# zhuzhui-2000/mobilesuperresolution

Measured on AMD Instinct MI355X. Metric: HR megapixels/sec (WDSR-B x4, 48x48 LR patches), full training step, higher is better.
Workload: dtype bf16; 1 GPU; WDSR-B x4, 16 blocks / 24 units, 48x48 LR patches, batch 32 per GPU, fwd+L1+bwd+Adam; global_batch=32, parallelism=dp1

## Files before the change

include/sr_hotpath.h:

```cpp
#ifndef SR_HOTPATH_H
#define SR_HOTPATH_H
#include <stddef.h>
#include <stdint.h>

#ifdef __cplusplus
extern "C" {
#endif

typedef void* sr_stream_t;

#define SR_DTYPE_F32 0
#define SR_DTYPE_BF16 1

int sr_abi_version(void);

int sr_wdsr_block_fwd(const void* x, void* y, const void* wblob, const float* cinit,
                      int N, int H, int W, int F, int dtype, sr_stream_t stream);

int sr_wdsr_block2_fwd(const void* x, void* ya, void* yb, const void* wblob_a, const void* wblob_b,
                       const float* cinit_a, const float* cinit_b, void* tsave_a, void* tsave_b, int N, int H, int W,
                       int F, int dtype, sr_stream_t stream);

int sr_wdsr_block2_bwd_data(const void* xa, const void* xb, const void* dyb, void* dxb, void* dxa,
                            const void* wblob_a, const void* wblob_b, const float* cinit_a, const float* cinit_b,
// ... 152 lines not shown
  const float* flat; float* gflat;
  const int* chan_tab; int n_chan;
  const int* bias_tab; const float* bias_const; int n_bias;
  float* src; float* dsrc;
  long src_head_off, src_body_off, src_body_stride, src_tail_off;
  const int* idx_head; int n_idx_head;
  const int* idx_body; int n_idx_body;
  const int* idx_cinit; int n_idx_cinit;
  const int* idx_tail; int n_idx_tail;
  void* blob_head; void* blob_body; float* cinit_body; void* blob_tail;
  float* part_a; float* part_b; float* part_tail; float* part_head;
  int wgs_body, wgs_tail, wgs_head;
  int slab_a, slab_b, slab_tail, slab_head;
  const int* ga_sidx; const int* ga_dst; int n_ga;
  const int* gb_sidx; const int* gb_dst; int n_gb;
  const int* gt_sidx; const int* gt_dst; int n_gt;
  const int* gh_sidx; const int* gh_dst; int n_gh;
  const float* x; void* acts; void* grads; float* out; const float* dout;
  void* tsave; void* dtsave;
  const float* hr; int loss_kind; float loss_gscale; float* loss_part;
  int nb_split, chan_split, bias_split;
  int adam_in_wn_bwd;
  int one_block32;
} sr_wdsr_net_t;

#define SR_NET_SAVE_ACTS 1
#define SR_NET_WEIGHTS_PACKED 2
#define SR_NET_PACK_ONLY 4
int sr_wdsr_net_forward(const sr_wdsr_net_t* net, int flags, sr_stream_t stream);
int sr_wdsr_net_backward(const sr_wdsr_net_t* net, sr_stream_t stream);
int sr_wdsr_net_backward_part(const sr_wdsr_net_t* net, int part, sr_stream_t stream);

int sr_pixel_shuffle(const float* in, float* out, int N, int C, int H, int W, int r, int inverse, sr_stream_t stream);

int sr_tail_bwd_loss(const float* sr, const float* hr, int loss_kind, float gscale, float* loss_part, const void* feat,
                     const float* x_nchw, float mean, const void* wblob, void* dfeat, float* partial, int wgs, int N, int H,
                     int W, int F, int R, int dtype, sr_stream_t stream);

typedef struct { float w_lerp, beta2, one_minus_beta2, bc2_sqrt, eps, neg_step_size; } sr_adam_t;
int sr_adam_step(float* param, const float* grad, float* exp_avg, float* exp_avg_sq, long n, const sr_adam_t* a,
                 const float* loss_part, int n_loss, float loss_scale, float* loss_out, sr_stream_t stream);
int sr_loss_value(const float* loss_part, int n_loss, float loss_scale, float* loss_out, sr_stream_t stream);
int sr_scale_by(void* y, const void* x, long n, const float* scale, int dtype, sr_stream_t stream);
int sr_wdsr_net_train_step(const sr_wdsr_net_t* net, float* exp_avg, float* exp_avg_sq, long n_params, const sr_adam_t* a,
                           float loss_scale, float* loss_out, sr_stream_t stream);

int sr_conv7_fwd(const void* x, const void* wpacked, const float* bias, void* y, int N, int H, int W, int CIN, int COUT, int relu,
                 int out_f32, sr_stream_t stream);

int sr_probe_mfma_bf16(const void* a_frag, const void* b_frag, float* acc_out, sr_stream_t stream);
int sr_probe_mfma_f32(const float* a_frag, const float* b_frag, float* acc_out, sr_stream_t stream);
int sr_probe_tr_read(const void* img_bf16, int n_elems, const int* lane_elem_off, void* out_bf16x4,
                     sr_stream_t stream);
int sr_probe_copy(const void* src, void* dst, size_t n_bytes, sr_stream_t stream);
int sr_probe_launch_floor(void* out, int gx, int gy, int threads, int lds_bytes, int reps, sr_stream_t stream);
int sr_probe_launch_floor_graph(void* out, int gx, int gy, int threads, int lds_bytes, int reps, int iters,
                                float* us_per_launch, float* host_us_per_graph );
int sr_debug_set_stamps(void* buf, long n_workgroups);

#ifdef __cplusplus
}
#endif
#endif
```

mobilesuperresolution_amd/_lib.py:

```python
from __future__ import annotations

import ctypes
import os
from ctypes import c_int, c_size_t, c_void_p

import torch

_HERE = os.path.dirname(os.path.abspath(__file__))
LIB_PATH = os.environ.get("SR_HOTPATH_LIB_PATH") or os.path.join(
    _HERE, "libsr_hotpath_dbg.so" if os.environ.get("SR_HOTPATH_DEBUG_LIB") == "1" else "libsr_hotpath.so")
ABI_VERSION = 17
DTYPE_CODE = {torch.float32: 0, torch.bfloat16: 1}

_P, _I, _Z, _L, _F = c_void_p, c_int, c_size_t, ctypes.c_long, ctypes.c_float
SIGNATURES = {
    "sr_abi_version": ([], _I),
    "sr_wdsr_block_fwd": ([_P, _P, _P, _P, _I, _I, _I, _I, _I, _P], _I),
    "sr_wdsr_block2_fwd": ([_P] * 9 + [_I] * 5 + [_P], _I),
    "sr_wdsr_fwd_rs": ([_P] * 9 + [_I] * 6 + [_P], _I),
    "sr_conv7_fwd": ([_P] * 4 + [_I] * 7 + [_P], _I),
    "sr_wdsr_fwd_rs_repeat": ([_P] * 9 + [_I] * 7 + [_P], _I),
    "sr_wdsr_block_wgrad_saved": ([_P] * 8 + [_I] * 7 + [_L] * 5 + [_P], _I),
    "sr_wdsr_block2_bwd_data": ([_P] * 11 + [_I] * 5 + [_P], _I),
    "sr_wdsr_block2_fwd_repeat": ([_P] * 7 + [_I] * 6 + [_P], _I),
    "sr_probe_launch_floor": ([_P, _I, _I, _I, _I, _I, _P], _I),
    "sr_probe_launch_floor_graph": ([_P, _I, _I, _I, _I, _I, _I, _P, _P], _I),
    "sr_debug_set_stamps": ([_P, _L], _I),
    "sr_c3_trunk_fwd": ([_P] * 6 + [_I] * 7 + [_L, _P], _I),
    "sr_c3_trunk_bwd": ([_P] * 11 + [_I] * 8 + [_L, _P], _I),
    "sr_c64_trunk_fwd": ([_P] * 7 + [_I] * 7 + [_L, _P], _I),
    "sr_tail_bwd": ([_P, _P, _P, _F, _P, _P, _P] + [_I] * 7 + [_P], _I),
    "sr_nas_dw_wgrad": ([_P, _P, _P, _P, _I, _I, _I, _I, _I, _I, _P], _I),
    "sr_wdsr_block_fwd_repeat": ([_P, _P, _P, _P, _I, _I, _I, _I, _I, _I, _P], _I),
    "sr_wdsr_block_bwd_data": ([_P, _P, _P, _P, _P, _I, _I, _I, _I, _I, _P], _I),
# ... 8 lines not shown
    "sr_c3_bwd_data": ([_P, _P, _P, _P, _P, _I, _I, _I, _I, _I, _I, _P], _I),
    "sr_c3_wgrad": ([_P, _P, _P, _P, _I, _I, _I, _I, _I, _I, _I, _P], _I),
    "sr_flow_warp_fwd": ([_P, _P, _P, _I, _I, _I, _I, _P], _I),
    "sr_flow_warp_bwd": ([_P, _P, _P, _P, _P, _I, _I, _I, _I, _P], _I),
    "sr_nas_dw_fwd": ([_P, _P, _P, _I, _I, _I, _I, _I, _P], _I),
    "sr_nas_pw_fwd": ([_P, _P, _P, _P, _P, _P, _I, _I, _I, _I, _I, _P], _I),
    "sr_nas_pw_bwd": ([_P, _P, _P, _P, _P, _P, _P, _P, _I, _I, _I, _I, _I, _I, _P], _I),
    "sr_nas_dw_bwd": ([_P, _P, _P, _P, _P, _P, _I, _I, _I, _I, _I, _I, _P], _I),
    "sr_patch_gather": ([_P, _P, _P, _P, _I, _I, _I, _P], _I),
    "sr_clip_gather": ([_P] * 7 + [_I] * 4 + [_P], _I),
    "sr_param_pack": ([_P, _P, _P, _I, _P, _P, _I, _P, _I, _I, _P], _I),
    "sr_param_grads": ([_P, _P, _P, _P, _I, _P, _I, _P, _I, _P], _I),
    "sr_nas_scalars": ([_P] * 5 + [_I, _I, _P, _P, _L, _I, _P, _P], _I),
    "sr_nas_mask_grads": ([_P, _L, _I, _I, _I, _I, _P, _P, _P, _I, _I, _P, _P], _I),
    "sr_nas_body_fwd": ([_P, _P, _P, _L, _P, _L, _P, _L, _P, _L] + [_I] * 7 + [_P], _I),
    "sr_nas_body_bwd": ([_P] * 7 + [_L, _P, _L, _P, _L, _P, _L, _P, _L, _P, _L] + [_I] * 8 + [_P, _P], _I),
    "sr_psnr": ([_P, _P, _P, _P] + [_I] * 7 + [_P], _I),
    "sr_pixel_shuffle": ([_P, _P, _I, _I, _I, _I, _I, _I, _P], _I),
    "sr_tail_bwd_loss": ([_P, _P, _I, _F, _P, _P, _P, _F, _P, _P, _P] + [_I] * 7 + [_P], _I),
    "sr_adam_step": ([_P, _P, _P, _P, _L, _P, _P, _I, _F, _P, _P], _I),
    "sr_loss_value": ([_P, _I, _F, _P, _P], _I),
    "sr_scale_by": ([_P, _P, _L, _P, _I, _P], _I),
    "sr_wdsr_net_train_step": ([_P, _P, _P, _L, _P, _F, _P, _P], _I),
    "sr_wdsr_net_forward": ([_P, _I, _P], _I),
    "sr_wdsr_net_backward": ([_P, _P], _I),
    "sr_wdsr_net_backward_part": ([_P, _I, _P], _I),
    "sr_probe_mfma_bf16": ([_P, _P, _P, _P], _I),
    "sr_probe_mfma_f32": ([_P, _P, _P, _P], _I),
    "sr_probe_tr_read": ([_P, _I, _P, _P, _P], _I),
    "sr_probe_copy": ([_P, _P, _Z, _P], _I),
    "sr_rm_block_fwd": ([_P] * 5 + [_I] * 6 + [_P], _I),
    "sr_rm_block_bwd_data": ([_P] * 4 + [_I] * 6 + [_P], _I),
    "sr_rm_wgrad": ([_P] * 4 + [_I] * 8 + [_P], _I),
    "sr_rm_tail_fwd": ([_P] * 3 + [_I] * 7 + [_P], _I),
    "sr_rm_unshuffle": ([_P, _P] + [_I] * 5 + [_P], _I),
    "sr_rm_tail_bwd_data": ([_P] * 3 + [_I] * 7 + [_P], _I),
}

class WdsrNet(ctypes.Structure):
    _fields_ = (
        [(n, _I) for n in ("F", "NB", "R", "dtype", "N", "H", "W")] + [("mean", _F)] +
        [("flat", _P), ("gflat", _P), ("chan_tab", _P), ("n_chan", _I),
         ("bias_tab", _P), ("bias_const", _P), ("n_bias", _I), ("src", _P), ("dsrc", _P)] +
        [(n, _L) for n in ("src_head_off", "src_body_off", "src_body_stride", "src_tail_off")] +
        [("idx_head", _P), ("n_idx_head", _I), ("idx_body", _P), ("n_idx_body", _I),
         ("idx_cinit", _P), ("n_idx_cinit", _I), ("idx_tail", _P), ("n_idx_tail", _I),
         ("blob_head", _P), ("blob_body", _P), ("cinit_body", _P), ("blob_tail", _P),
         ("part_a", _P), ("part_b", _P), ("part_tail", _P), ("part_head", _P)] +
        [(n, _I) for n in ("wgs_body", "wgs_tail", "wgs_head", "slab_a", "slab_b", "slab_tail", "slab_head")] +
        [("ga_sidx", _P), ("ga_dst", _P), ("n_ga", _I), ("gb_sidx", _P), ("gb_dst", _P), ("n_gb", _I),
         ("gt_sidx", _P), ("gt_dst", _P), ("n_gt", _I), ("gh_sidx", _P), ("gh_dst", _P), ("n_gh", _I),
         ("x", _P), ("acts", _P), ("grads", _P), ("out", _P), ("dout", _P), ("tsave", _P), ("dtsave", _P),
         ("hr", _P), ("loss_kind", _I), ("loss_gscale", _F), ("loss_part", _P),
         ("nb_split", _I), ("chan_split", _I), ("bias_split", _I), ("adam_in_wn_bwd", _I),
         ("one_block32", _I)])


class C3Warp(ctypes.Structure):
    _fields_ = [("frame", _P), ("frame_bs", _L), ("state", _P), ("flow", _P), ("flow_bs", _L), ("flow_bound", _P),
                ("dstate", _P), ("dflow", _P), ("dflow_bs", _L), ("x0_save", _P)]


class C3Unpack(ctypes.Structure):
    _fields_ = [("sidx0", _P), ("dst0", _P), ("n0", _I), ("sidx1", _P), ("dst1", _P), ("n1", _I), ("gflat", _P)]


class PackSeg(ctypes.Structure):
    _fields_ = [("idx", _P), ("out", _P), ("src_off", _L), ("src_stride", _L), ("n", _I), ("reps", _I), ("as_float", _I)]


class UnpackSeg(ctypes.Structure):
    _fields_ = [("partial", _P), ("sidx", _P), ("dst", _P), ("dst_off", _L), ("dst_stride", _L), ("slab", _L), ("wgs", _I),
                ("n", _I), ("reps", _I)]


class AdamScalars(ctypes.Structure):
    _fields_ = [(n, _F) for n in ("w_lerp", "beta2", "one_minus_beta2", "bc2_sqrt", "eps", "neg_step_size")]

# ... 102 lines not shown
```

mobilesuperresolution_amd/csrc/sr_abi.hip:

```cpp
#include <algorithm>
#include "../../include/sr_hotpath.h"
#include "wdsr_block.h"
#include "wdsr_fwd_rs.h"
#include "wdsr_fwd_stream.h"
#include "wdsr_bwd_rs.h"
#include "wdsr_bwd_pair_lds.h"
#include "wdsr_wgrad_rs.h"
#include "wdsr_ends.h"
#include "wdsr_prep.h"
#include "conv3x3.h"
#include "conv64.h"
#include "spynet_conv.h"
#include "nas_block.h"
#include "nas_dw_lc.h"
#include "nas_bwd_fused.h"
#include "flow_warp.h"
#include "metrics.h"
#include "patches.h"
#include "clips.h"
#include "train_step.h"
#include "pixel_shuffle.h"
#include "result_block.h"

extern "C" int sr_abi_version(void) { return 17; }

namespace {

template <typename T, int F, int E, int L>
int launch_block_fwd(const void* x, void* y, const void* wblob, const float* cinit, int N, int H, int W,
                     hipStream_t st, void* tsave = nullptr) {
  typedef BlockCfg<F, E, L> C;
  const int tiles_x = (W + C::TW - 1) / C::TW, tiles_y = (H + C::TH - 1) / C::TH;
  dim3 grid(tiles_x * tiles_y, N), block(64 * C::NPT_H);
  hipLaunchKernelGGL((wdsr_block_fwd_kernel<T, F, E, L>), grid, block, 0, st, (const T*)x, (T*)y, (const T*)wblob,
                     cinit, H, W, tiles_x, (T*)tsave);
  SR_HIP_CHECK_LAUNCH();
  return 0;
}

template <typename T, int F, int E, int L>
int launch_block_bwd_data(const void* x, const void* dy, void* dx, const void* wblob, const float* cinit, int N,
                          int H, int W, hipStream_t st, void* dtsave = nullptr) {
  typedef BlockCfg<F, E, L> C;
  const int tiles_x = (W + C::TW - 1) / C::TW, tiles_y = (H + C::TH - 1) / C::TH;
  dim3 grid(tiles_x * tiles_y, N), block(64 * C::NPT_O);
  hipLaunchKernelGGL((wdsr_block_bwd_data_kernel<T, F, E, L>), grid, block, 0, st, (const T*)x, (const T*)dy, (T*)dx,
                     (const T*)wblob, cinit, H, W, tiles_x, (T*)dtsave);
// ... 857 lines not shown
        return rc;
      cur = nxt;
      continue;
    }
    if (save_acts && saved) {
      rc = n->F == 24 ? launch_block_fwd<__bf16, 24, 144, 20>(cur, nxt, (char*)n->blob_body + i * blob,
                                                              n->cinit_body + (size_t)i * n->n_idx_cinit, n->N, n->H, n->W,
                                                              st, (char*)n->tsave + (size_t)i * side)
                      : launch_block_fwd<__bf16, 32, 192, 26>(cur, nxt, (char*)n->blob_body + i * blob,
                                                              n->cinit_body + (size_t)i * n->n_idx_cinit, n->N, n->H, n->W,
                                                              st, (char*)n->tsave + (size_t)i * side);
      if (rc) return rc;
    } else if ((rc = sr_wdsr_block_fwd(cur, nxt, (char*)n->blob_body + i * blob,
                                       n->cinit_body + (size_t)i * n->n_idx_cinit, n->N, n->H, n->W, n->F, n->dtype, stream)))
      return rc;
    cur = nxt;
  }
  return sr_tail_fwd(cur, n->x, n->out, n->blob_tail, n->mean, n->N, n->H, n->W, n->F, n->R, n->dtype, stream);
}

namespace {
struct FusedAdam { float* m; float* v; AdamArgs a; const float* loss_part; int n_loss; float loss_scale; float* loss_out; };
}
static int net_backward_part_impl(const sr_wdsr_net_t* n, int part, sr_stream_t stream, const FusedAdam* fa) {
  if (!n || !n->flat || !n->gflat || !n->dsrc || !n->x || !n->acts || !n->grads || part < 0 || part > 2) return -2;
  if (part != 2 && (n->hr ? (!n->out || !n->loss_part || (n->loss_kind != 1 && n->loss_kind != 2)) : !n->dout)) return -2;
  hipStream_t st = (hipStream_t)stream;
  const size_t esz = n->dtype == SR_DTYPE_BF16 ? 2 : 4;
  const size_t act = (size_t)n->N * n->H * n->W * n->F * esz;
  const size_t blob = (size_t)n->n_idx_body * esz;
  const long act_e = (long)n->N * n->H * n->W * n->F;
  char* acts = (char*)n->acts;
  char* grads = (char*)n->grads;
  const bool pairs = net_uses_pairs(n);
  const bool saved = net_saves_side_images(n, true);
  const size_t side = side_image_bytes(n);
  int split = part == 0 ? 0 : n->nb_split;
  if (part != 0 && (split <= 0 || split >= n->NB || (pairs && ((n->NB - split) & 1)))) return -2;
  const int b0 = part == 1 ? split : 0, b1 = part == 2 ? split : n->NB;
  int rc;
  if (part != 2) {
    if (n->hr) {
      if ((rc = sr_tail_bwd_loss(n->out, n->hr, n->loss_kind, n->loss_gscale, n->loss_part, acts + (size_t)n->NB * act, n->x,
                                 n->mean, n->blob_tail, grads + (size_t)n->NB * act, n->part_tail, n->wgs_tail, n->N, n->H, n->W,
                                 n->F, n->R, n->dtype, stream)))
        return rc;
// ... 41 lines not shown
      return rc;
  }
  const int nl = b1 - b0;
  const int wgs_part = nl > 0 ? (n->wgs_body * n->NB) / nl : 0;
  if (nl > 0) {
    char* a0 = acts + (size_t)b0 * act;
    char* g1 = grads + (size_t)(b0 + 1) * act;
    char* wb0 = (char*)n->blob_body + (size_t)b0 * blob;
    const float* ci0 = n->cinit_body + (size_t)b0 * n->n_idx_cinit;
    float* pa0 = n->part_a;
    float* pb0 = n->part_b;
    if (saved) {
      if ((rc = sr_wdsr_block_wgrad_saved(a0, g1, (char*)n->tsave + (size_t)b0 * side, (char*)n->dtsave + (size_t)b0 * side, wb0, ci0,
                                          pa0, pb0, nl, wgs_part, n->N, n->H, n->W, n->F, n->dtype, act_e, act_e,
                                          (long)(side / esz), (long)n->n_idx_body, (long)n->n_idx_cinit, stream)))
        return rc;
    } else if ((rc = sr_wdsr_block_wgrad(a0, g1, wb0, ci0, pa0, pb0, nl, wgs_part, n->N, n->H, n->W, n->F, n->dtype, act_e,
                                         act_e, (long)n->n_idx_body, (long)n->n_idx_cinit, stream)))
      return rc;
  }
  if (part != 1)
    if ((rc = sr_head_wgrad(grads, n->x, n->mean, n->part_head, n->wgs_head, n->N, n->H, n->W, n->F, n->dtype, stream)))
      return rc;
  {
    UnpackSegs us;
    us.nseg = 0;
    int blk = 0;
    auto add = [&](const float* part_, const int* sidx, const int* dst, long off, long stride, long slab, int wgs, int cnt,
                   int reps) {
      us.s[us.nseg++] = UnpackSeg{part_, sidx, dst, off, stride, slab, wgs, cnt, reps, blk};
      blk += reps * unpack_blocks(cnt, wgs);
    };
    if (nl > 0) {
      add(n->part_a, n->ga_sidx, n->ga_dst, n->src_body_off + b0 * n->src_body_stride, n->src_body_stride, n->slab_a, wgs_part,
          n->n_ga, nl);
      add(n->part_b, n->gb_sidx, n->gb_dst, n->src_body_off + b0 * n->src_body_stride, n->src_body_stride, n->slab_b, wgs_part,
          n->n_gb, nl);
    }
    if (part != 2) add(n->part_tail, n->gt_sidx, n->gt_dst, n->src_tail_off, 0, n->slab_tail, n->wgs_tail, n->n_gt, 1);
    if (part != 1) add(n->part_head, n->gh_sidx, n->gh_dst, n->src_head_off, 0, n->slab_head, n->wgs_head, n->n_gh, 1);
    hipLaunchKernelGGL(unpack_all_kernel, dim3(blk), dim3(64 * UNPACK_Q), 0, st, n->dsrc, us);
  }
  const int c0 = part == 1 ? n->chan_split : 0, c1 = part == 2 ? n->chan_split : n->n_chan;
  const int d0 = part == 1 ? n->bias_split : 0, d1 = part == 2 ? n->bias_split : n->n_bias;
  const int cb = (c1 - c0 + 3) / 4, bb = (d1 - d0 + 255) / 256;
  if (fa)
    hipLaunchKernelGGL(wn_bwd_adam_kernel, dim3(cb + bb), dim3(256), 0, st, const_cast<float*>(n->flat), n->dsrc, n->gflat, fa->m, fa->v,
                       (const int4*)n->chan_tab + c0, c1 - c0, n->bias_tab + 3 * d0, d1 - d0, cb, fa->a, fa->loss_part, fa->n_loss,
                       fa->loss_scale, fa->loss_out);
  else
    hipLaunchKernelGGL(wn_bwd_kernel, dim3(cb + bb), dim3(256), 0, st, n->flat, n->dsrc, n->gflat, (const int4*)n->chan_tab + c0,
                       c1 - c0, n->bias_tab + 3 * d0, d1 - d0, cb);
  SR_HIP_CHECK_LAUNCH();
  return 0;
}
extern "C" int sr_wdsr_net_backward_part(const sr_wdsr_net_t* n, int part, sr_stream_t stream) {
  return net_backward_part_impl(n, part, stream, nullptr);
}

extern "C" int sr_wdsr_net_backward(const sr_wdsr_net_t* n, sr_stream_t stream) { return sr_wdsr_net_backward_part(n, 0, stream); }

extern "C" int sr_param_pack(const float* flat, float* src, const int* chan_tab, int n_chan, const int* bias_tab,
                             const float* bias_const, int n_bias, const sr_pack_seg_t* segs, int nseg, int dtype,
                             sr_stream_t stream) {
  if (!flat || !src || !chan_tab || n_chan <= 0 || n_bias < 0 || (n_bias > 0 && (!bias_tab || !bias_const)) || !segs || nseg < 1 ||
      nseg > 4 || (dtype != SR_DTYPE_F32 && dtype != SR_DTYPE_BF16))
    return -2;
  hipStream_t st = (hipStream_t)stream;
  const int cb = (n_chan + 3) / 4, bb = (n_bias + 255) / 256;
  hipLaunchKernelGGL(wn_src_kernel, dim3(cb + bb), dim3(256), 0, st, flat, src, (const int4*)chan_tab, n_chan, bias_tab, bias_const,
                     n_bias, cb);
  PackSegs ps;
  ps.nseg = nseg;
  int blk = 0;
  for (int k = 0; k < nseg; ++k) {
    const sr_pack_seg_t& g = segs[k];
    if (!g.idx || !g.out || g.n <= 0 || g.reps <= 0) return -2;
// ... 210 lines not shown
extern "C" int sr_scale_by(void* y, const void* x, long n, const float* scale, int dtype, sr_stream_t stream) {
  if (!y || !x || !scale || n <= 0 || ((uintptr_t)y & 15) || ((uintptr_t)x & 15)) return -2;
  const unsigned blocks = (unsigned)((n + 2047) / 2048);
  if (dtype == SR_DTYPE_BF16)
    hipLaunchKernelGGL(scale_by_kernel<__bf16>, dim3(blocks), dim3(256), 0, (hipStream_t)stream, (__bf16*)y, (const __bf16*)x, n, scale);
  else if (dtype == SR_DTYPE_F32)
    hipLaunchKernelGGL(scale_by_kernel<float>, dim3(blocks), dim3(256), 0, (hipStream_t)stream, (float*)y, (const float*)x, n, scale);
  else return -1;
  SR_HIP_CHECK_LAUNCH();
  return 0;
}
extern "C" int sr_wdsr_net_train_step(const sr_wdsr_net_t* n, float* m, float* v, long n_params, const sr_adam_t* a,
                                      float loss_scale, float* loss_out, sr_stream_t stream) {
  if (!n || !n->hr || !m || !v || !a || n_params <= 0) return -2;
  int rc;
  if ((rc = sr_wdsr_net_forward(n, SR_NET_SAVE_ACTS, stream))) return rc;
  if (n->adam_in_wn_bwd) {
    const FusedAdam fa{m, v, AdamArgs{a->w_lerp, a->beta2, a->one_minus_beta2, a->bc2_sqrt, a->eps, a->neg_step_size}, n->loss_part,
                       n->wgs_tail, loss_scale, loss_out};
    return net_backward_part_impl(n, 0, stream, &fa);
  }
  if ((rc = sr_wdsr_net_backward(n, stream))) return rc;
  return sr_adam_step(const_cast<float*>(n->flat), n->gflat, m, v, n_params, a, n->loss_part, n->wgs_tail, loss_scale, loss_out, stream);
}

__global__ void probe_mfma_bf16_kernel(const bf16x8* a, const bf16x8* b, float* out) {
  const int l = threadIdx.x;
  f32x16 acc = zero16();
  acc = mma16<__bf16>(a[l], b[l], acc);
#pragma unroll
  for (int i = 0; i < 16; ++i) out[l * 16 + i] = acc[i];
}
__global__ void probe_mfma_f32_kernel(const f32x8* a, const f32x8* b, float* out) {
  const int l = threadIdx.x;
  f32x16 acc = zero16();
  acc = mma16<float>(a[l], b[l], acc);
#pragma unroll
  for (int i = 0; i < 16; ++i) out[l * 16 + i] = acc[i];
}
__global__ void probe_tr_kernel(const __bf16* img, int n, const int* off, bf16x4* out) {
  __shared__ __attribute__((aligned(16))) __bf16 lds[8192];
  for (int i = threadIdx.x; i < n && i < 8192; i += 64) lds[i] = img[i];
  __syncthreads();
  typedef __attribute__((address_space(3))) bf16x4 lds_bf16x4;
  out[threadIdx.x] = __builtin_amdgcn_ds_read_tr16_b64_v4bf16((lds_bf16x4*)(lds + off[threadIdx.x]));
}
// ... 258 lines not shown
```

mobilesuperresolution_amd/csrc/train_step.h:

```cpp
#pragma once
#include "sr_common.h"

struct AdamArgs {
  float w_lerp, beta2, one_minus_beta2, bc2_sqrt, eps, neg_step_size;
};
__global__ __launch_bounds__(256) void adam_step_kernel(float* __restrict__ p, const float* __restrict__ g,
                                                        float* __restrict__ m, float* __restrict__ v, long n, AdamArgs a,
                                                        const float* __restrict__ loss_part, int n_loss, float loss_scale,
                                                        float* __restrict__ loss_out) {
  const long i0 = ((long)blockIdx.x * 256 + threadIdx.x) * 4;
  if (i0 + 3 < n) {
    const f32x4 gv = *reinterpret_cast<const f32x4*>(g + i0);
    f32x4 mv = *reinterpret_cast<const f32x4*>(m + i0), vv = *reinterpret_cast<const f32x4*>(v + i0);
    f32x4 pv = *reinterpret_cast<const f32x4*>(p + i0);
#pragma unroll
    for (int j = 0; j < 4; ++j) {
      mv[j] = __builtin_fmaf(a.w_lerp, gv[j] - mv[j], mv[j]);
      const float vb = vv[j] * a.beta2;
      vv[j] = __builtin_fmaf(a.one_minus_beta2, gv[j] * gv[j], vb);
      const float d = __builtin_sqrtf(vv[j]) / a.bc2_sqrt + a.eps;
      pv[j] = __builtin_fmaf(a.neg_step_size, mv[j] / d, pv[j]);
    }
    *reinterpret_cast<f32x4*>(m + i0) = mv;
    *reinterpret_cast<f32x4*>(v + i0) = vv;
// ... 30 lines not shown
template <typename T>
__global__ __launch_bounds__(256) void scale_by_kernel(T* __restrict__ y, const T* __restrict__ x, long n, const float* __restrict__ scale) {
  const float s = *scale;
  const long i0 = ((long)blockIdx.x * 256 + threadIdx.x) * 8;
  if (i0 + 8 <= n) {
    typedef T V __attribute__((ext_vector_type(8)));
    V v = *reinterpret_cast<const V*>(x + i0);
#pragma unroll
    for (int j = 0; j < 8; ++j) v[j] = (T)((float)v[j] * s);
    *reinterpret_cast<V*>(y + i0) = v;
  } else {
    for (long i = i0; i < n; ++i) y[i] = (T)((float)x[i] * s);
  }
}

SR_DEV void adam_elem(float& p, float g, float& m, float& v, const AdamArgs& a) {
  m = __builtin_fmaf(a.w_lerp, g - m, m);
  const float vb = v * a.beta2;
  v = __builtin_fmaf(a.one_minus_beta2, g * g, vb);
  const float d = __builtin_sqrtf(v) / a.bc2_sqrt + a.eps;
  p = __builtin_fmaf(a.neg_step_size, m / d, p);
}

__global__ __launch_bounds__(256) void wn_bwd_adam_kernel(float* __restrict__ flat, const float* __restrict__ dsrc,
                                                          float* __restrict__ gflat, float* __restrict__ em, float* __restrict__ ev,
                                                          const int4* __restrict__ chan_tab, int n_chan,
                                                          const int* __restrict__ bias_tab, int n_bias, int chan_blocks, AdamArgs a,
                                                          const float* __restrict__ loss_part, int n_loss, float loss_scale,
                                                          float* __restrict__ loss_out) {
  const int lane = threadIdx.x & 63, wave = threadIdx.x >> 6;
  if (loss_out && blockIdx.x == gridDim.x - 1 && threadIdx.x >= 192) {
    float s = 0.f;
    for (int i = lane; i < n_loss; i += 64) s += loss_part[i];
#pragma unroll
    for (int o = 32; o > 0; o >>= 1) s += __shfl_xor(s, o);
    if (lane == 0) *loss_out = s * loss_scale;
  }
  if ((int)blockIdx.x < chan_blocks) {
    const int c = blockIdx.x * 4 + wave;
    if (c >= n_chan) return;
    const int4 t = chan_tab[c];
    float* v = flat + t.x;
    const float* dw = dsrc + t.w;
    float ss = 0.f, dot = 0.f;
    for (int k = lane; k < t.z; k += 64) { const float x = v[k]; ss += x * x; dot += x * dw[k]; }
#pragma unroll
    for (int o = 32; o > 0; o >>= 1) { ss += __shfl_xor(ss, o); dot += __shfl_xor(dot, o); }
    const float n = sqrtf(ss), g = flat[t.y];
    const float s1 = g / n, s2 = dot / ss;
    for (int k = lane; k < t.z; k += 64) {
      float gk = s1 * (dw[k] - v[k] * s2);
      asm volatile("" : "+v"(gk));
      gflat[t.x + k] = gk;
      float pk = v[k], mk = em[t.x + k], vk = ev[t.x + k];
      adam_elem(pk, gk, mk, vk, a);
      v[k] = pk; em[t.x + k] = mk; ev[t.x + k] = vk;
    }
    if (lane == 0) {
      float gg = dot / n;
      asm volatile("" : "+v"(gg));
      gflat[t.y] = gg;
      float pg = g, mg = em[t.y], vg = ev[t.y];
      adam_elem(pg, gg, mg, vg, a);
      flat[t.y] = pg; em[t.y] = mg; ev[t.y] = vg;
    }
  } else {
    const int i = (blockIdx.x - chan_blocks) * 256 + threadIdx.x;
    if (i >= n_bias) return;
    const int pa = bias_tab[3 * i], pb = bias_tab[3 * i + 1], d = bias_tab[3 * i + 2];
    const float gval = dsrc[d];
    gflat[pa] = gval;
    { float pp = flat[pa], mm = em[pa], vv = ev[pa]; adam_elem(pp, gval, mm, vv, a); flat[pa] = pp; em[pa] = mm; ev[pa] = vv; }
    if (pb >= 0) {
      gflat[pb] = gval;
      float pp = flat[pb], mm = em[pb], vv = ev[pb];
      adam_elem(pp, gval, mm, vv, a);
      flat[pb] = pp; em[pb] = mm; ev[pb] = vv;
    }
  }
}
```

mobilesuperresolution_amd/layout.py:

```python
from __future__ import annotations

from collections import OrderedDict
from dataclasses import dataclass
from functools import lru_cache

import numpy as np

from . import packing as P


@dataclass(frozen=True)
class ConvSpec:
    name: str
    cout: int
    cin: int
    k: int


class WDSRLayout:
    def __init__(self, F: int, NB: int, R: int):
        self.F, self.NB, self.R = F, NB, R
        E, L = int(F * 6), int(F * 0.84)
        self.E, self.L = E, L
        CO = 3 * R * R
# ... 73 lines not shown
        self.idx_cinit = bt_["cinit"].astype(np.int32)

        gt = P.block_grad_tables(F, E, L)
        n_w1, n_w2, n_w3 = E * F, L * E, F * L * 9
        ga, gb = gt["a"], gt["b"]
        dst_a = np.concatenate([ob["w1"] + np.arange(n_w1), ob["w2"] + np.arange(n_w2),
                                ob["b1"] + np.arange(E), ob["b2"] + np.arange(L)])
        dst_b = np.concatenate([ob["w3"] + np.arange(n_w3), ob["b3"] + np.arange(F)])
        def by_slab(sidx, dst):
            o = np.argsort(sidx, kind="stable")
            return sidx[o].astype(np.int32), dst[o].astype(np.int32)
        self.ga = by_slab(ga, dst_a)
        self.gb = by_slab(gb, dst_b)
        self.slab_a, self.slab_b = gt["a_size"], gt["b_size"]
        ge = P.ends_grad_tables(F, R)
        n_t = CO * F * 9 + CO * 75 + CO
        dst_t = np.concatenate([ot["wt"] + np.arange(CO * F * 9), ot["ws"] + np.arange(CO * 75),
                                ot["b"] + np.arange(CO)])
        assert ge["tail"].size == n_t
        self.gt = by_slab(ge["tail"], dst_t)
        dst_h = np.concatenate([oh["wh"] + np.arange(F * 27), oh["b"] + np.arange(F)])
        self.gh = by_slab(ge["head"], dst_h)
        self.slab_tail, self.slab_head = ge["tail_size"], ge["head_size"]


    def split_at(self, nb_split: int):
        per_block = sum(c.cout for c in self.convs if c.name.startswith("body.0."))
        head_rows = next(c.cout for c in self.convs if c.name == "head")
        first = min(off for name, (off, _) in self.entries.items() if name.startswith(f"body.{nb_split}."))
        return first, head_rows + nb_split * per_block, head_rows + nb_split * per_block


@lru_cache(maxsize=None)
def get_layout(F: int, NB: int, R: int) -> WDSRLayout:
    return WDSRLayout(F, NB, R)
```

mobilesuperresolution_amd/models/basic_wdsr_b.py:

```python
from __future__ import annotations

import ctypes
import math
import os
from collections import OrderedDict

import numpy as np
import torch
import torch.nn as nn

from .. import _lib as L
from ..layout import get_layout

__all__ = ["BASIC_MODEL"]

_DTYPES = {"fp32": torch.float32, "float32": torch.float32, "bf16": torch.bfloat16, "bfloat16": torch.bfloat16}


def _hot_dtype(params) -> torch.dtype:
    name = getattr(params, "hot_dtype", None) or os.environ.get("SR_HOT_DTYPE", "fp32")
    if isinstance(name, torch.dtype):
        return name
    return _DTYPES[str(name).lower()]

# ... 38 lines not shown
            setattr(n, "idx_" + k, self.idx[k].data_ptr())
            setattr(n, "n_idx_" + k, self.idx[k].numel())
        n.blob_head, n.blob_body = self.blob_head.data_ptr(), self.blob_body.data_ptr()
        n.cinit_body, n.blob_tail = self.cinit_body.data_ptr(), self.blob_tail.data_ptr()
        n.part_a, n.part_b = self.part_a.data_ptr(), self.part_b.data_ptr()
        n.part_tail, n.part_head = self.part_tail.data_ptr(), self.part_head.data_ptr()
        n.wgs_body, n.wgs_tail, n.wgs_head = self.wgs_body, self.wgs_tail, self.wgs_head
        n.slab_a, n.slab_b, n.slab_tail, n.slab_head = lay.slab_a, lay.slab_b, lay.slab_tail, lay.slab_head
        for k in ("ga", "gb", "gt", "gh"):
            setattr(n, k + "_sidx", self.g[k][0].data_ptr())
            setattr(n, k + "_dst", self.g[k][1].data_ptr())
            setattr(n, "n_" + k, self.g[k][0].numel())
        n.loss_part = self.loss_part.data_ptr()
        ct, bt = lay.chan_tab, lay.bias_tab
        cover = np.zeros(int(model.flat.numel()), dtype=np.int32)
        for v_off, g_off, K, _dst in ct:
            cover[v_off:v_off + K] += 1
            cover[g_off] += 1
        for a_, b_, _d in bt:
            cover[a_] += 1
            if b_ >= 0:
                cover[b_] += 1
        n.adam_in_wn_bwd = int(bool((cover == 1).all()))
        n.one_block32 = int(model.one_block32)
        if model.nb_split:
            _, n.chan_split, n.bias_split = lay.split_at(model.nb_split)
            n.nb_split = model.nb_split
        self.net = n

    def call_struct(self) -> "L.WdsrNet":
        return L.WdsrNet.from_buffer_copy(self.net)


class BASIC_MODEL(nn.Module):

    def __init__(self, params):
        super().__init__()
        self.image_mean = float(params.image_mean)
        self.scale = int(params.scale)
        self.remain_blocks = params.num_blocks
        nin = int(params.num_channels)
        f = int(params.num_residual_units)
        nb = int(params.num_blocks)
        self.num_residual_units, self.num_blocks = f, nb
        if nin != 3 or f not in (24, 32) or self.scale not in (2, 3, 4) or nb < 1:
            raise NotImplementedError(
# ... 491 lines not shown
```

Baseline: 3574 HR-Mpix/s.

## Fuse slab unpack with weight-norm backward and Adam into one grouped kernel

Adds a param_grads_adam_kernel that reduces the per-workgroup gradient slabs, applies the weight-norm backward, and runs the Adam update in one launch per parameter group. The reduced gradients are staged in LDS instead of being re-read from dsrc. Host-side layout code builds per-group tables (rows, biases, slab element indices) and passes them through new fields in the net struct. This removes one launch and a global-memory round trip between unpack and Adam. The cost is more complex per-group indexing and one 1024-thread block per group, which could limit parallelism for large layers.

```diff
diff --git a/include/sr_hotpath.h b/include/sr_hotpath.h
--- a/include/sr_hotpath.h
+++ b/include/sr_hotpath.h
@@ -198,6 +198,7 @@
   int nb_split, chan_split, bias_split;
   int adam_in_wn_bwd;
   int one_block32;
+  const int* pg_groups; int n_pg_groups; const int* pg_elems; int pg_max_elems;
 } sr_wdsr_net_t;
 
 #define SR_NET_SAVE_ACTS 1
@@ -220,6 +221,8 @@
 int sr_scale_by(void* y, const void* x, long n, const float* scale, int dtype, sr_stream_t stream);
 int sr_wdsr_net_train_step(const sr_wdsr_net_t* net, float* exp_avg, float* exp_avg_sq, long n_params, const sr_adam_t* a,
                            float loss_scale, float* loss_out, sr_stream_t stream);
+int sr_wdsr_net_param_step(const sr_wdsr_net_t* net, float* exp_avg, float* exp_avg_sq, const sr_adam_t* a, float loss_scale,
+                           float* loss_out, int fused, sr_stream_t stream);
 
 int sr_conv7_fwd(const void* x, const void* wpacked, const float* bias, void* y, int N, int H, int W, int CIN, int COUT, int relu,
                  int out_f32, sr_stream_t stream);
diff --git a/mobilesuperresolution_amd/_lib.py b/mobilesuperresolution_amd/_lib.py
--- a/mobilesuperresolution_amd/_lib.py
+++ b/mobilesuperresolution_amd/_lib.py
@@ -9,7 +9,7 @@
 _HERE = os.path.dirname(os.path.abspath(__file__))
 LIB_PATH = os.environ.get("SR_HOTPATH_LIB_PATH") or os.path.join(
     _HERE, "libsr_hotpath_dbg.so" if os.environ.get("SR_HOTPATH_DEBUG_LIB") == "1" else "libsr_hotpath.so")
-ABI_VERSION = 17
+ABI_VERSION = 18
 DTYPE_CODE = {torch.float32: 0, torch.bfloat16: 1}
 
 _P, _I, _Z, _L, _F = c_void_p, c_int, c_size_t, ctypes.c_long, ctypes.c_float
@@ -64,6 +64,7 @@
     "sr_loss_value": ([_P, _I, _F, _P, _P], _I),
     "sr_scale_by": ([_P, _P, _L, _P, _I, _P], _I),
     "sr_wdsr_net_train_step": ([_P, _P, _P, _L, _P, _F, _P, _P], _I),
+    "sr_wdsr_net_param_step": ([_P, _P, _P, _P, _F, _P, _I, _P], _I),
     "sr_wdsr_net_forward": ([_P, _I, _P], _I),
     "sr_wdsr_net_backward": ([_P, _P], _I),
     "sr_wdsr_net_backward_part": ([_P, _I, _P], _I),
@@ -95,7 +96,7 @@
          ("x", _P), ("acts", _P), ("grads", _P), ("out", _P), ("dout", _P), ("tsave", _P), ("dtsave", _P),
          ("hr", _P), ("loss_kind", _I), ("loss_gscale", _F), ("loss_part", _P),
          ("nb_split", _I), ("chan_split", _I), ("bias_split", _I), ("adam_in_wn_bwd", _I),
-         ("one_block32", _I)])
+         ("one_block32", _I), ("pg_groups", _P), ("n_pg_groups", _I), ("pg_elems", _P), ("pg_max_elems", _I)])
 
 
 class C3Warp(ctypes.Structure):
diff --git a/mobilesuperresolution_amd/csrc/sr_abi.hip b/mobilesuperresolution_amd/csrc/sr_abi.hip
--- a/mobilesuperresolution_amd/csrc/sr_abi.hip
+++ b/mobilesuperresolution_amd/csrc/sr_abi.hip
@@ -22,7 +22,7 @@
 #include "pixel_shuffle.h"
 #include "result_block.h"
 
-extern "C" int sr_abi_version(void) { return 17; }
+extern "C" int sr_abi_version(void) { return 18; }
 
 namespace {
 
@@ -926,6 +926,52 @@
 namespace {
 struct FusedAdam { float* m; float* v; AdamArgs a; const float* loss_part; int n_loss; float loss_scale; float* loss_out; };
 }
+static int net_param_grads(const sr_wdsr_net_t* n, int part, int b0, int nl, int wgs_part, hipStream_t st, const FusedAdam* fa,
+                           bool fused) {
+  if (fused) {
+    if (!fa || part != 0 || !n->pg_groups || !n->pg_elems || n->n_pg_groups <= 0) return -2;
+    if (n->pg_max_elems > PG_LDS) return -1;
+    SlabSrc ss{{n->part_a, n->part_b, n->part_tail, n->part_head},
+               {n->slab_a, n->slab_b, n->slab_tail, n->slab_head},
+               {n->wgs_body, n->wgs_body, n->wgs_tail, n->wgs_head}};
+    hipLaunchKernelGGL(param_grads_adam_kernel, dim3(n->n_pg_groups), dim3(PG_THREADS), 0, st, const_cast<float*>(n->flat), n->dsrc,
+                       n->gflat, fa->m, fa->v, (const int4*)n->chan_tab, n->bias_tab, (const int4*)n->pg_groups,
+                       (const int2*)n->pg_elems, ss, fa->a, fa->loss_part, fa->n_loss, fa->loss_scale, fa->loss_out);
+    SR_HIP_CHECK_LAUNCH();
+    return 0;
+  }
+  {
+    UnpackSegs us;
+    us.nseg = 0;
+    int blk = 0;
+    auto add = [&](const float* part_, const int* sidx, const int* dst, long off, long stride, long slab, int wgs, int cnt,
+                   int reps) {
+      us.s[us.nseg++] = UnpackSeg{part_, sidx, dst, off, stride, slab, wgs, cnt, reps, blk};
+      blk += reps * unpack_blocks(cnt, wgs);
+    };
+    if (nl > 0) {
+      add(n->part_a, n->ga_sidx, n->ga_dst, n->src_body_off + b0 * n->src_body_stride, n->src_body_stride, n->slab_a, wgs_part,
+          n->n_ga, nl);
+      add(n->part_b, n->gb_sidx, n->gb_dst, n->src_body_off + b0 * n->src_body_stride, n->src_body_stride, n->slab_b, wgs_part,
+          n->n_gb, nl);
+    }
+    if (part != 2) add(n->part_tail, n->gt_sidx, n->gt_dst, n->src_tail_off, 0, n->slab_tail, n->wgs_tail, n->n_gt, 1);
+    if (part != 1) add(n->part_head, n->gh_sidx, n->gh_dst, n->src_head_off, 0, n->slab_head, n->wgs_head, n->n_gh, 1);
+    hipLaunchKernelGGL(unpack_all_kernel, dim3(blk), dim3(64 * UNPACK_Q), 0, st, n->dsrc, us);
+  }
+  const int c0 = part == 1 ? n->chan_split : 0, c1 = part == 2 ? n->chan_split : n->n_chan;
+  const int d0 = part == 1 ? n->bias_split : 0, d1 = part == 2 ? n->bias_split : n->n_bias;
+  const int cb = (c1 - c0 + 3) / 4, bb = (d1 - d0 + 255) / 256;
+  if (fa)
+    hipLaunchKernelGGL(wn_bwd_adam_kernel, dim3(cb + bb), dim3(256), 0, st, const_cast<float*>(n->flat), n->dsrc, n->gflat, fa->m, fa->v,
+                       (const int4*)n->chan_tab + c0, c1 - c0, n->bias_tab + 3 * d0, d1 - d0, cb, fa->a, fa->loss_part, fa->n_loss,
+                       fa->loss_scale, fa->loss_out);
+  else
+    hipLaunchKernelGGL(wn_bwd_kernel, dim3(cb + bb), dim3(256), 0, st, n->flat, n->dsrc, n->gflat, (const int4*)n->chan_tab + c0,
+                       c1 - c0, n->bias_tab + 3 * d0, d1 - d0, cb);
+  SR_HIP_CHECK_LAUNCH();
+  return 0;
+}
 static int net_backward_part_impl(const sr_wdsr_net_t* n, int part, sr_stream_t stream, const FusedAdam* fa) {
   if (!n || !n->flat || !n->gflat || !n->dsrc || !n->x || !n->acts || !n->grads || part < 0 || part > 2) return -2;
   if (part != 2 && (n->hr ? (!n->out || !n->loss_part || (n->loss_kind != 1 && n->loss_kind != 2)) : !n->dout)) return -2;
@@ -1013,37 +1059,7 @@
   if (part != 1)
     if ((rc = sr_head_wgrad(grads, n->x, n->mean, n->part_head, n->wgs_head, n->N, n->H, n->W, n->F, n->dtype, stream)))
       return rc;
-  {
-    UnpackSegs us;
-    us.nseg = 0;
-    int blk = 0;
-    auto add = [&](const float* part_, const int* sidx, const int* dst, long off, long stride, long slab, int wgs, int cnt,
-                   int reps) {
-      us.s[us.nseg++] = UnpackSeg{part_, sidx, dst, off, stride, slab, wgs, cnt, reps, blk};
-      blk += reps * unpack_blocks(cnt, wgs);
-    };
-    if (nl > 0) {
-      add(n->part_a, n->ga_sidx, n->ga_dst, n->src_body_off + b0 * n->src_body_stride, n->src_body_stride, n->slab_a, wgs_part,
-          n->n_ga, nl);
-      add(n->part_b, n->gb_sidx, n->gb_dst, n->src_body_off + b0 * n->src_body_stride, n->src_body_stride, n->slab_b, wgs_part,
-          n->n_gb, nl);
-    }
-    if (part != 2) add(n->part_tail, n->gt_sidx, n->gt_dst, n->src_tail_off, 0, n->slab_tail, n->wgs_tail, n->n_gt, 1);
-    if (part != 1) add(n->part_head, n->gh_sidx, n->gh_dst, n->src_head_off, 0, n->slab_head, n->wgs_head, n->n_gh, 1);
-    hipLaunchKernelGGL(unpack_all_kernel, dim3(blk), dim3(64 * UNPACK_Q), 0, st, n->dsrc, us);
-  }
-  const int c0 = part == 1 ? n->chan_split : 0, c1 = part == 2 ? n->chan_split : n->n_chan;
-  const int d0 = part == 1 ? n->bias_split : 0, d1 = part == 2 ? n->bias_split : n->n_bias;
-  const int cb = (c1 - c0 + 3) / 4, bb = (d1 - d0 + 255) / 256;
-  if (fa)
-    hipLaunchKernelGGL(wn_bwd_adam_kernel, dim3(cb + bb), dim3(256), 0, st, const_cast<float*>(n->flat), n->dsrc, n->gflat, fa->m, fa->v,
-                       (const int4*)n->chan_tab + c0, c1 - c0, n->bias_tab + 3 * d0, d1 - d0, cb, fa->a, fa->loss_part, fa->n_loss,
-                       fa->loss_scale, fa->loss_out);
-  else
-    hipLaunchKernelGGL(wn_bwd_kernel, dim3(cb + bb), dim3(256), 0, st, n->flat, n->dsrc, n->gflat, (const int4*)n->chan_tab + c0,
-                       c1 - c0, n->bias_tab + 3 * d0, d1 - d0, cb);
-  SR_HIP_CHECK_LAUNCH();
-  return 0;
+  return net_param_grads(n, part, b0, nl, wgs_part, st, fa, fa != nullptr);
 }
 extern "C" int sr_wdsr_net_backward_part(const sr_wdsr_net_t* n, int part, sr_stream_t stream) {
   return net_backward_part_impl(n, part, stream, nullptr);
@@ -1300,6 +1316,15 @@
   }
   if ((rc = sr_wdsr_net_backward(n, stream))) return rc;
   return sr_adam_step(const_cast<float*>(n->flat), n->gflat, m, v, n_params, a, n->loss_part, n->wgs_tail, loss_scale, loss_out, stream);
+}
+
+extern "C" int sr_wdsr_net_param_step(const sr_wdsr_net_t* n, float* m, float* v, const sr_adam_t* a, float loss_scale,
+                                      float* loss_out, int fused, sr_stream_t stream) {
+  if (!n || !n->flat || !n->gflat || !n->dsrc || !m || !v || !a || !n->adam_in_wn_bwd || (loss_out && !n->loss_part)) return -2;
+  if (!n->part_a || !n->part_b || !n->part_tail || !n->part_head) return -2;
+  const FusedAdam fa{m, v, AdamArgs{a->w_lerp, a->beta2, a->one_minus_beta2, a->bc2_sqrt, a->eps, a->neg_step_size}, n->loss_part,
+                     n->wgs_tail, loss_scale, loss_out};
+  return net_param_grads(n, 0, 0, n->NB, n->wgs_body, (hipStream_t)stream, &fa, fused != 0);
 }
 
 __global__ void probe_mfma_bf16_kernel(const bf16x8* a, const bf16x8* b, float* out) {
diff --git a/mobilesuperresolution_amd/csrc/train_step.h b/mobilesuperresolution_amd/csrc/train_step.h
--- a/mobilesuperresolution_amd/csrc/train_step.h
+++ b/mobilesuperresolution_amd/csrc/train_step.h
@@ -76,6 +76,51 @@
   p = __builtin_fmaf(a.neg_step_size, m / d, p);
 }
 
+SR_DEV void wn_row_adam(float* __restrict__ flat, const float* dw, float* __restrict__ gflat, float* __restrict__ em,
+                        float* __restrict__ ev, const int4 t, const int lane, const AdamArgs& a) {
+  float* v = flat + t.x;
+  float ss = 0.f, dot = 0.f;
+  for (int k = lane; k < t.z; k += 64) { const float x = v[k]; ss += x * x; dot += x * dw[k]; }
+#pragma unroll
+  for (int o = 32; o > 0; o >>= 1) { ss += __shfl_xor(ss, o); dot += __shfl_xor(dot, o); }
+  const float n = sqrtf(ss), g = flat[t.y];
+  const float s1 = g / n, s2 = dot / ss;
+  for (int k = lane; k < t.z; k += 64) {
+    float gk = s1 * (dw[k] - v[k] * s2);
+    asm volatile("" : "+v"(gk));
+    gflat[t.x + k] = gk;
+    float pk = v[k], mk = em[t.x + k], vk = ev[t.x + k];
+    adam_elem(pk, gk, mk, vk, a);
+    v[k] = pk; em[t.x + k] = mk; ev[t.x + k] = vk;
+  }
+  if (lane == 0) {
+    float gg = dot / n;
+    asm volatile("" : "+v"(gg));
+    gflat[t.y] = gg;
+    float pg = g, mg = em[t.y], vg = ev[t.y];
+    adam_elem(pg, gg, mg, vg, a);
+    flat[t.y] = pg; em[t.y] = mg; ev[t.y] = vg;
+  }
+}
+SR_DEV void bias_adam(float* __restrict__ flat, const float gval, float* __restrict__ gflat, float* __restrict__ em,
+                      float* __restrict__ ev, const int pa, const int pb, const AdamArgs& a) {
+  gflat[pa] = gval;
+  { float pp = flat[pa], mm = em[pa], vv = ev[pa]; adam_elem(pp, gval, mm, vv, a); flat[pa] = pp; em[pa] = mm; ev[pa] = vv; }
+  if (pb >= 0) {
+    gflat[pb] = gval;
+    float pp = flat[pb], mm = em[pb], vv = ev[pb];
+    adam_elem(pp, gval, mm, vv, a);
+    flat[pb] = pp; em[pb] = mm; ev[pb] = vv;
+  }
+}
+SR_DEV void loss_fold(const float* __restrict__ loss_part, int n_loss, float loss_scale, float* __restrict__ loss_out, int lane) {
+  float s = 0.f;
+  for (int i = lane; i < n_loss; i += 64) s += loss_part[i];
+#pragma unroll
+  for (int o = 32; o > 0; o >>= 1) s += __shfl_xor(s, o);
+  if (lane == 0) *loss_out = s * loss_scale;
+}
+
 __global__ __launch_bounds__(256) void wn_bwd_adam_kernel(float* __restrict__ flat, const float* __restrict__ dsrc,
                                                           float* __restrict__ gflat, float* __restrict__ em, float* __restrict__ ev,
                                                           const int4* __restrict__ chan_tab, int n_chan,
@@ -83,53 +128,150 @@
                                                           const float* __restrict__ loss_part, int n_loss, float loss_scale,
                                                           float* __restrict__ loss_out) {
   const int lane = threadIdx.x & 63, wave = threadIdx.x >> 6;
-  if (loss_out && blockIdx.x == gridDim.x - 1 && threadIdx.x >= 192) {
-    float s = 0.f;
-    for (int i = lane; i < n_loss; i += 64) s += loss_part[i];
-#pragma unroll
-    for (int o = 32; o > 0; o >>= 1) s += __shfl_xor(s, o);
-    if (lane == 0) *loss_out = s * loss_scale;
-  }
+  if (loss_out && blockIdx.x == gridDim.x - 1 && threadIdx.x >= 192)
+    loss_fold(loss_part, n_loss, loss_scale, loss_out, lane);
   if ((int)blockIdx.x < chan_blocks) {
     const int c = blockIdx.x * 4 + wave;
     if (c >= n_chan) return;
     const int4 t = chan_tab[c];
-    float* v = flat + t.x;
-    const float* dw = dsrc + t.w;
+    wn_row_adam(flat, dsrc + t.w, gflat, em, ev, t, lane, a);
+  } else {
+    const int i = (blockIdx.x - chan_blocks) * 256 + threadIdx.x;
+    if (i >= n_bias) return;
+    bias_adam(flat, dsrc[bias_tab[3 * i + 2]], gflat, em, ev, bias_tab[3 * i], bias_tab[3 * i + 1], a);
+  }
+}
+
+struct SlabSrc { const float* part[4]; long slab[4]; int wgs[4]; };
+constexpr int PG_THREADS = 1024, PG_Q = 16, PG_J = 4;
+constexpr int PG_LDS = 2048;
+constexpr int PG_ROWS = 64;
+__global__ __launch_bounds__(PG_THREADS) void param_grads_adam_kernel(float* __restrict__ flat, float* __restrict__ dsrc,
+                                                                      float* __restrict__ gflat, float* __restrict__ em,
+                                                                      float* __restrict__ ev, const int4* __restrict__ chan_tab,
+                                                                      const int* __restrict__ bias_tab, const int4* __restrict__ grp_tab,
+                                                                      const int2* __restrict__ elem_tab, SlabSrc src, AdamArgs a,
+                                                                      const float* __restrict__ loss_part, int n_loss, float loss_scale,
+                                                                      float* __restrict__ loss_out) {
+  __shared__ float dw[PG_LDS], vs[PG_LDS];
+  __shared__ float red[PG_Q][64 * PG_J];
+  __shared__ float rs1[PG_ROWS], rs2[PG_ROWS];
+  const int tid = threadIdx.x, lane = tid & 63, wave = tid >> 6;
+  if (loss_out && blockIdx.x == gridDim.x - 1 && wave == PG_Q - 1)
+    loss_fold(loss_part, n_loss, loss_scale, loss_out, lane);
+  const int4 g0 = grp_tab[3 * blockIdx.x], g1 = grp_tab[3 * blockIdx.x + 1], g2 = grp_tab[3 * blockIdx.x + 2];
+  const int kind = g0.x, ntab = g0.w, row0 = g1.x, nrows = g1.y, bias0 = g1.z, nbias = g1.w;
+  const int K = g2.x, nw = nrows * K;
+  const long w_dst = g2.y, v0 = g2.z, b_dst = g2.w;
+  float pv0 = 0.f, mk0 = 0.f, vk0 = 0.f;
+  if (tid < nw) { pv0 = flat[v0 + tid]; mk0 = em[v0 + tid]; vk0 = ev[v0 + tid]; }
+  int g_off0 = 0;
+  float gp0 = 0.f, gm0 = 0.f, gv0 = 0.f;
+  if (wave < nrows) {
+    g_off0 = chan_tab[row0 + wave].y;
+    gp0 = flat[g_off0]; gm0 = em[g_off0]; gv0 = ev[g_off0];
+  }
+  const float* part = kind == 0 ? src.part[0] : kind == 1 ? src.part[1] : kind == 2 ? src.part[2] : src.part[3];
+  const long slab = kind == 0 ? src.slab[0] : kind == 1 ? src.slab[1] : kind == 2 ? src.slab[2] : src.slab[3];
+  const int wgs = kind == 0 ? src.wgs[0] : kind == 1 ? src.wgs[1] : kind == 2 ? src.wgs[2] : src.wgs[3];
+  const float* const base = part + (size_t)g0.y * wgs * slab;
+  const int2* const tab = elem_tab + g0.z;
+  auto put = [&](int local, float v) {
+    dw[local] = v;
+    dsrc[local < nw ? w_dst + local : b_dst + (local - nw)] = v;
+  };
+  if (wgs == PG_Q) {
+    for (int j = tid; j < ntab; j += PG_THREADS) {
+      const int2 e = tab[j];
+      float x[PG_Q];
+#pragma unroll
+      for (int w = 0; w < PG_Q; ++w) x[w] = (base + (size_t)w * slab)[(unsigned)e.x];
+      float v = 0.f;
+#pragma unroll
+      for (int w = 0; w < PG_Q; ++w) v += x[w];
+      put(e.y, v);
+    }
+  } else if (wgs <= 4 * PG_Q) {
+    for (int j = tid; j < ntab; j += PG_THREADS) {
+      const int2 e = tab[j];
+      float v = 0.f;
+      for (int q = 0; q < PG_Q; ++q) {
+        float r = 0.f;
+        for (int w = q; w < wgs; w += PG_Q) r += (base + (size_t)w * slab)[(unsigned)e.x];
+        v += r;
+      }
+      put(e.y, v);
+    }
+  } else {
+    for (int p0 = 0; p0 < ntab; p0 += 64 * PG_J) {
+      float acc[PG_J];
+      unsigned p[PG_J];
+#pragma unroll
+      for (int j = 0; j < PG_J; ++j) {
+        acc[j] = 0.f;
+        p[j] = tab[min(p0 + lane + 64 * j, ntab - 1)].x;
+      }
+      int w = __builtin_amdgcn_readfirstlane(wave);
+      for (; w + 15 * PG_Q < wgs; w += 16 * PG_Q) {
+        float x[16][PG_J];
+#pragma unroll
+        for (int u = 0; u < 16; ++u)
+#pragma unroll
+          for (int j = 0; j < PG_J; ++j) x[u][j] = (base + (size_t)(w + u * PG_Q) * slab)[p[j]];
+#pragma unroll
+        for (int u = 0; u < 16; ++u)
+#pragma unroll
+          for (int j = 0; j < PG_J; ++j) acc[j] += x[u][j];
+      }
+      for (; w < wgs; w += PG_Q) {
+#pragma unroll
+        for (int j = 0; j < PG_J; ++j) acc[j] += (base + (size_t)w * slab)[p[j]];
+      }
+#pragma unroll
+      for (int j = 0; j < PG_J; ++j) red[wave][lane + 64 * j] = acc[j];
+      __syncthreads();
+      if (tid < 64 * PG_J && p0 + tid < ntab) {
+        float v = 0.f;
+#pragma unroll
+        for (int q = 0; q < PG_Q; ++q) v += red[q][tid];
+        put(tab[p0 + tid].y, v);
+      }
+      __syncthreads();
+    }
+  }
+  for (int i = tid; i < nw; i += PG_THREADS) vs[i] = i == tid ? pv0 : flat[v0 + i];
+  __syncthreads();
+  for (int r = wave; r < nrows; r += PG_Q) {
+    const float* v = vs + r * K;
+    const float* d = dw + r * K;
     float ss = 0.f, dot = 0.f;
-    for (int k = lane; k < t.z; k += 64) { const float x = v[k]; ss += x * x; dot += x * dw[k]; }
+    for (int k = lane; k < K; k += 64) { const float x = v[k]; ss += x * x; dot += x * d[k]; }
 #pragma unroll
     for (int o = 32; o > 0; o >>= 1) { ss += __shfl_xor(ss, o); dot += __shfl_xor(dot, o); }
-    const float n = sqrtf(ss), g = flat[t.y];
-    const float s1 = g / n, s2 = dot / ss;
-    for (int k = lane; k < t.z; k += 64) {
-      float gk = s1 * (dw[k] - v[k] * s2);
-      asm volatile("" : "+v"(gk));
-      gflat[t.x + k] = gk;
-      float pk = v[k], mk = em[t.x + k], vk = ev[t.x + k];
-      adam_elem(pk, gk, mk, vk, a);
-      v[k] = pk; em[t.x + k] = mk; ev[t.x + k] = vk;
-    }
+    const bool first = r == wave;
+    const int g_off = first ? g_off0 : chan_tab[row0 + r].y;
+    const float n = sqrtf(ss), g = first ? gp0 : flat[g_off];
     if (lane == 0) {
+      rs1[r] = g / n;
+      rs2[r] = dot / ss;
       float gg = dot / n;
       asm volatile("" : "+v"(gg));
-      gflat[t.y] = gg;
-      float pg = g, mg = em[t.y], vg = ev[t.y];
+      gflat[g_off] = gg;
+      float pg = g, mg = first ? gm0 : em[g_off], vg = first ? gv0 : ev[g_off];
       adam_elem(pg, gg, mg, vg, a);
-      flat[t.y] = pg; em[t.y] = mg; ev[t.y] = vg;
-    }
-  } else {
-    const int i = (blockIdx.x - chan_blocks) * 256 + threadIdx.x;
-    if (i >= n_bias) return;
-    const int pa = bias_tab[3 * i], pb = bias_tab[3 * i + 1], d = bias_tab[3 * i + 2];
-    const float gval = dsrc[d];
-    gflat[pa] = gval;
-    { float pp = flat[pa], mm = em[pa], vv = ev[pa]; adam_elem(pp, gval, mm, vv, a); flat[pa] = pp; em[pa] = mm; ev[pa] = vv; }
-    if (pb >= 0) {
-      gflat[pb] = gval;
-      float pp = flat[pb], mm = em[pb], vv = ev[pb];
-      adam_elem(pp, gval, mm, vv, a);
-      flat[pb] = pp; em[pb] = mm; ev[pb] = vv;
-    }
-  }
-}
+      flat[g_off] = pg; em[g_off] = mg; ev[g_off] = vg;
+    }
+  }
+  __syncthreads();
+  for (int i = tid; i < nw; i += PG_THREADS) {
+    const int r = i / K;
+    const float s1 = rs1[r], s2 = rs2[r];
+    float pk = vs[i], mk = i == tid ? mk0 : em[v0 + i], vk = i == tid ? vk0 : ev[v0 + i];
+    float gk = s1 * (dw[i] - pk * s2);
+    asm volatile("" : "+v"(gk));
+    gflat[v0 + i] = gk;
+    adam_elem(pk, gk, mk, vk, a);
+    flat[v0 + i] = pk; em[v0 + i] = mk; ev[v0 + i] = vk;
+  }
+  if (tid < nbias) bias_adam(flat, dw[nw + tid], gflat, em, ev, bias_tab[3 * (bias0 + tid)], bias_tab[3 * (bias0 + tid) + 1], a);
+}
diff --git a/mobilesuperresolution_amd/layout.py b/mobilesuperresolution_amd/layout.py
--- a/mobilesuperresolution_amd/layout.py
+++ b/mobilesuperresolution_amd/layout.py
@@ -119,6 +119,71 @@
         dst_h = np.concatenate([oh["wh"] + np.arange(F * 27), oh["b"] + np.arange(F)])
         self.gh = by_slab(ge["head"], dst_h)
         self.slab_tail, self.slab_head = ge["tail_size"], ge["head_size"]
+        self.pg_groups, self.pg_elems = self._param_groups()
+
+    PG_KINDS = ("ga", "gb", "gt", "gh")
+    PG_MAX_ELEMS, PG_MAX_ROWS = 2048, 64
+
+    def _param_groups(self):
+        F, NB, E, L, CO = self.F, self.NB, self.E, self.L, self.CO
+        ob, ot, oh = self.block_geom.off, self.ends_geom.tail_off, self.ends_geom.head_off
+        sizes = {"ga": ob["size"], "gb": ob["size"], "gt": ot["size"], "gh": oh["size"]}
+        inv = {}
+        for k in self.PG_KINDS:
+            sidx, dst = getattr(self, k)
+            a = np.full(sizes[k], -1, dtype=np.int64)
+            assert np.unique(dst).size == dst.size
+            a[dst] = sidx
+            inv[k] = a
+        seg_base = {"ga": None, "gb": None, "gt": self.src_tail_off, "gh": self.src_head_off}
+        bias_row = {int(d): i for i, (_a, _b, d) in enumerate(self.bias_tab)}
+        groups, elems, shared = [], [], {}
+        n_elems = 0
+
+        def conv_groups(row0, cout, kind, layer, key):
+            nonlocal n_elems
+            K = int(self.chan_tab[row0, 2])
+            base = self.src_body_off + layer * self.src_body_stride if seg_base[kind] is None else seg_base[kind]
+            many = kind in ("gt", "gh")
+            G = 1 if many else max(1, 1 << int(np.log2(max(1, 1024 // K))))
+            for r0 in range(0, cout, G):
+                g = min(G, cout - r0)
+                w_dst = int(self.chan_tab[row0 + r0, 3])
+                v_off = int(self.chan_tab[row0 + r0, 0])
+                assert all(int(self.chan_tab[row0 + r0 + r, 3]) == w_dst + r * K for r in range(g))
+                assert all(int(self.chan_tab[row0 + r0 + r, 0]) == v_off + r * K for r in range(g))
+                assert g <= self.PG_MAX_ROWS and g * K <= 1024
+                b0, nb_ = 0, 0
+                if key[1] is not None:
+                    b_dst = key[1] + r0
+                    b0, nb_ = bias_row[base + b_dst], g
+                    assert all(bias_row[base + b_dst + j] == b0 + j for j in range(g))
+                if (key, r0) not in shared:
+                    rel = np.concatenate([np.arange(w_dst - base, w_dst - base + g * K),
+                                          np.arange(key[1] + r0, key[1] + r0 + nb_) if nb_ else np.zeros(0, dtype=np.int64)]).astype(np.int64)
+                    sidx = inv[kind][rel]
+                    assert (sidx >= 0).all(), "an element of a weight-norm row that no slab feeds"
+                    o = np.argsort(sidx, kind="stable")
+                    assert rel.size <= self.PG_MAX_ELEMS
+                    shared[(key, r0)] = (n_elems, rel.size)
+                    elems.append(np.stack([sidx[o], np.arange(rel.size)[o]], axis=1))
+                    n_elems += rel.size
+                t0, nt = shared[(key, r0)]
+                groups.append((self.PG_KINDS.index(kind), layer if seg_base[kind] is None else 0, t0, nt, row0 + r0, g, b0, nb_,
+                               K, w_dst, v_off, base + key[1] + r0 if nb_ else 0))
+
+        row = 0
+        conv_groups(row, F, "gh", 0, ("head", oh["b"])); row += F
+        for i in range(NB):
+            conv_groups(row, E, "ga", i, ("w1", ob["b1"])); row += E
+            conv_groups(row, L, "ga", i, ("w2", ob["b2"])); row += L
+            conv_groups(row, F, "gb", i, ("w3", ob["b3"])); row += F
+        conv_groups(row, CO, "gt", 0, ("tail", ot["b"])); row += CO
+        conv_groups(row, CO, "gt", 0, ("skip", None)); row += CO
+        assert row == self.chan_tab.shape[0]
+        groups = np.asarray(groups, dtype=np.int32)
+        groups = groups[np.argsort(np.choose(groups[:, 0], [2, 2, 0, 1]), kind="stable")]
+        return groups, np.concatenate(elems).astype(np.int32)
 
 
     def split_at(self, nb_split: int):
diff --git a/mobilesuperresolution_amd/models/basic_wdsr_b.py b/mobilesuperresolution_amd/models/basic_wdsr_b.py
--- a/mobilesuperresolution_amd/models/basic_wdsr_b.py
+++ b/mobilesuperresolution_amd/models/basic_wdsr_b.py
@@ -84,6 +84,9 @@
             if b_ >= 0:
                 cover[b_] += 1
         n.adam_in_wn_bwd = int(bool((cover == 1).all()))
+        self.pg_groups, self.pg_elems = t(lay.pg_groups), t(lay.pg_elems)
+        n.pg_groups, n.n_pg_groups = self.pg_groups.data_ptr(), lay.pg_groups.shape[0]
+        n.pg_elems, n.pg_max_elems = self.pg_elems.data_ptr(), int(lay.pg_groups[:, 3].max())
         n.one_block32 = int(model.one_block32)
         if model.nb_split:
             _, n.chan_split, n.bias_split = lay.split_at(model.nb_split)
```

Measured after the change: 3576 HR-Mpix/s (median of 2 runs). Within noise of the previous version (+0.1%).
